# Sapphire-Bridge/rag-foundation

Hardware: AMD Instinct MI355X
Metric: top-k retrieval QPS + achieved HBM GB/s, 10M×768 k=10, 1/2/4/8 MI355X (higher is better)
Workload: dtype bf16; 1 GPU; cfg3: 10000000x768 bf16 corpus row-sharded over 1 GPU(s), 256 queries/batch, brute-force top-10; rows=10000000, dim=768, nq=256, k=10, parallelism=rowshard1, corpus_copies=1, scan=auto, exchange=none (one shard)

## Files before the change

rag-foundation_amd/csrc/k10_dbg.hip:

```cpp
#define RFX_K10_BLOCK_TIMES
#include "k_scan_screen64.h"

namespace rfx {
namespace k10q {
int launch_768(int kl, dim3 grid, hipStream_t st, const int8_t* X, const uint4* tm, const uint32_t* sts, const int8_t* Qc,
               const float* qe2, int nq, int ntiles, uint32_t* tau, float* cs, int* cr, uint32_t* dr, int64_t n_lists,
               const uint32_t* mask, uint32_t* xb, uint32_t* xw);
}

int launch_scan_screen_dbg(const MfmaPlan& p, int variant, const int8_t* X, const void* tmv, const uint32_t* sts,
                           int nrows, const int8_t* Qc, const float* qe2, int nq, uint32_t* tau, float* cs, int* cr,
                           uint32_t* dr, hipStream_t st) {
  const uint4* tm = (const uint4*)tmv;
  if (!p.ok || p.k_lane != 10) return -1;
  const int ntiles = (nrows + k10::kTM - 1) / k10::kTM;
  dim3 grid(p.blocks, p.q_blocks);
#define RFX_K10V(R, M)                                                                                        \
  case 100000000 * R + M:                                                                                          \
    hipLaunchKernelGGL((k10::scan_screen_kernel<10, 768, false, R, M>), grid, dim3(512), 0, st, X, tm, sts, Qc, \
                       qe2, nq, ntiles, tau, cs, cr, dr, p.n_lists, nullptr, tau + p.nq_pad * k10::kTauW,      \
                       xcd_weights_device_ptr());                                                             \
    break;
  switch (variant) {
    RFX_K10V(10, 2097152 + 8388608)
    RFX_K10V(10, 2097152 + 8388608 + 1)
    RFX_K10V(10, 2097152 + 8388608 + 9)
    RFX_K10V(10, 2097152 + 8388608 + 512)
    RFX_K10V(10, 2097152 + 8388608 + 8192)
    RFX_K10V(10, 2097152 + 8388608 + 65536)
    RFX_K10V(10, 2097152 + 8388608 + 33554432)
    case 64:
      if (p.lists_per_block != 1) return -1;
      return k10q::launch_768(10, grid, st, X, tm, sts, Qc, qe2, nq, ntiles, tau, cs, cr, dr, p.n_lists, nullptr,
                              tau + p.nq_pad * k10::kTauW, xcd_weights_device_ptr());
    case 65:
    case 73:
      if (p.lists_per_block != 1) return -1;
      if (variant == 65)
        hipLaunchKernelGGL((k10q::scan_screen_q64_kernel<10, 768, false, k10q::kRing768, 1>), grid, dim3(256), 0, st, X,
                           tm, sts, Qc, qe2, nq, ntiles, tau, cs, cr, dr, p.n_lists, nullptr, tau + p.nq_pad * k10::kTauW,
                           xcd_weights_device_ptr());
      else
        hipLaunchKernelGGL((k10q::scan_screen_q64_kernel<10, 768, false, k10q::kRing768, 9>), grid, dim3(256), 0, st, X,
                           tm, sts, Qc, qe2, nq, ntiles, tau, cs, cr, dr, p.n_lists, nullptr, tau + p.nq_pad * k10::kTauW,
                           xcd_weights_device_ptr());
      break;
    default:
      return -1;
  }
#undef RFX_K10V
  return 0;
}

int dbg_k10_trips(unsigned int* out_h, int reset) {
  if (reset) {
    static const unsigned int z[2][64] = {};
    return hipMemcpyToSymbol(HIP_SYMBOL(k10::g_k10_trips), z, sizeof(z)) == hipSuccess ? 0 : -1;
  }
  return hipMemcpyFromSymbol(out_h, HIP_SYMBOL(k10::g_k10_trips), sizeof(k10::g_k10_trips)) == hipSuccess ? 0 : -1;
}

int dbg_k10_block_times(unsigned long long* out_h) {
  return hipMemcpyFromSymbol(out_h, HIP_SYMBOL(k10::g_k10_bt), sizeof(k10::g_k10_bt)) == hipSuccess ? 0 : -1;
}

}
```

rag-foundation_amd/csrc/k_mfma_common.h:

```cpp
#pragma once
#include "rfx_device.h"
#include "rfx_kernels.h"

namespace rfx {
namespace mfc {

typedef __attribute__((ext_vector_type(8))) __bf16 v4bf16x8;
typedef __attribute__((ext_vector_type(8))) _Float16 v4f16x8;
typedef __attribute__((ext_vector_type(16))) float v4f32x16;

template <int DT>
__device__ __forceinline__ v4f32x16 mfma(const uint4& a, const uint4& b, const v4f32x16& c) {
  if constexpr (DT == RFX_BF16)
    return __builtin_amdgcn_mfma_f32_32x32x16_bf16(__builtin_bit_cast(v4bf16x8, a), __builtin_bit_cast(v4bf16x8, b),
                                                   c, 0, 0, 0);
  else
    return __builtin_amdgcn_mfma_f32_32x32x16_f16(__builtin_bit_cast(v4f16x8, a), __builtin_bit_cast(v4f16x8, b), c,
                                                  0, 0, 0);
}

typedef __attribute__((ext_vector_type(4))) float v4f32x4;
template <int DT>
__device__ __forceinline__ v4f32x4 mfma16(const uint4& a, const uint4& b, const v4f32x4& c) {
  if constexpr (DT == RFX_BF16)
    return __builtin_amdgcn_mfma_f32_16x16x32_bf16(__builtin_bit_cast(v4bf16x8, a), __builtin_bit_cast(v4bf16x8, b),
                                                   c, 0, 0, 0);
  else
    return __builtin_amdgcn_mfma_f32_16x16x32_f16(__builtin_bit_cast(v4f16x8, a), __builtin_bit_cast(v4f16x8, b), c,
                                                  0, 0, 0);
}

__device__ __forceinline__ uint32_t ord(float f) {
  const uint32_t b = __float_as_uint(f);
  return (b & 0x80000000u) ? ~b : (b | 0x80000000u);
}
__device__ __forceinline__ float unord(uint32_t o) {
  return __uint_as_float((o & 0x80000000u) ? (o & 0x7fffffffu) : ~o);
}
__device__ __forceinline__ float max3f(float a, float b, float c) { return fmaxf(fmaxf(a, b), c); }

typedef int v4i32 __attribute__((ext_vector_type(4)));

__device__ __forceinline__ v4i32 make_rsrc(const void* base) {
  const uint64_t a = (uint64_t)(uintptr_t)base;
  v4i32 d;
  d.x = __builtin_amdgcn_readfirstlane((int)(uint32_t)a);
  d.y = __builtin_amdgcn_readfirstlane((int)(uint32_t)(a >> 32) & 0xffff);
  d.z = -1;
  d.w = 0x00020000;
  return d;
}
__device__ __forceinline__ void bdma(v4i32 rsrc, uint32_t voff, uint32_t lds_addr) {
  asm volatile("s_nop 4\n\ts_mov_b32 m0, %2\n\ts_nop 0\n\tbuffer_load_dwordx4 %0, %1, 0 offen lds" ::"v"(voff), "s"(rsrc),
               "s"(lds_addr)
               : "memory", "m0");
}
__device__ __forceinline__ void bdma_nt(v4i32 rsrc, uint32_t voff, uint32_t lds_addr) {
  asm volatile("s_nop 4\n\ts_mov_b32 m0, %2\n\ts_nop 0\n\tbuffer_load_dwordx4 %0, %1, 0 offen nt lds" ::"v"(voff),
               "s"(rsrc), "s"(lds_addr)
               : "memory", "m0");
}
__device__ __forceinline__ void bdma_sc1(v4i32 rsrc, uint32_t voff, uint32_t lds_addr) {
  asm volatile("s_nop 4\n\ts_mov_b32 m0, %2\n\ts_nop 0\n\tbuffer_load_dwordx4 %0, %1, 0 offen sc1 lds" ::"v"(voff),
               "s"(rsrc), "s"(lds_addr)
               : "memory", "m0");
}
__device__ __forceinline__ void batomic_umax(v4i32 rsrc, uint32_t voff, uint32_t val) {
  asm volatile("s_nop 4\n\tbuffer_atomic_umax %0, %1, %2, 0 offen" ::"v"(val), "v"(voff), "s"(rsrc) : "memory");
}

__device__ __forceinline__ void glds(const void* src, uint32_t lds_addr) {
  asm volatile("s_mov_b32 m0, %1\n\ts_nop 0\n\tglobal_load_lds_dwordx4 %0, off" ::"v"(src), "s"(lds_addr)
               : "memory", "m0");
}
__device__ __forceinline__ void glds_sc1(const void* src, uint32_t lds_addr) {
  asm volatile("s_mov_b32 m0, %1\n\ts_nop 0\n\tglobal_load_lds_dwordx4 %0, off sc1" ::"v"(src), "s"(lds_addr)
               : "memory", "m0");
}

template <int N>
__device__ __forceinline__ void launder(uint4 (&v)[N]) {
#pragma unroll
  for (int i = 0; i < N; ++i) {
    v4i32 t = __builtin_bit_cast(v4i32, v[i]);
    asm volatile("" : "+v"(t));
    v[i] = __builtin_bit_cast(uint4, t);
  }
}

struct Acc4View {
  const v4f32x4 (&a)[4];
  __device__ __forceinline__ float operator[](int r) const { return a[r >> 2][r & 3]; }
};

template <int KL>
__device__ __forceinline__ uint32_t tau_min(const uint8_t* p) {
  const uint4 a = *(const uint4*)p;
  uint32_t m = min(min(a.x, a.y), min(a.z, a.w));
  if constexpr (KL > 4) {
    const uint4 b = *(const uint4*)(p + 16), c = *(const uint4*)(p + 32);
    m = min(m, min(min(b.x, b.y), min(b.z, b.w)));
    m = min(m, min(c.x, c.y));
  }
  return m;
}

template <int KL, int ROWMAP = 0, class V = v4f32x16>
__device__ __forceinline__ void fold(const V& acc, uint64_t* Ls, uint32_t& thr_o, int rbase, v4i32 tau_rsrc,
                                     uint32_t slot_voff, int& n_slow) {
  float mx = max3f(acc[0], acc[1], acc[2]);
#pragma unroll
  for (int r = 3; r < 15; r += 2) mx = max3f(mx, acc[r], acc[r + 1]);
  mx = fmaxf(mx, acc[15]);
  const float thr = thr_o ? unord(thr_o) : -__builtin_inff();
  if (mx >= thr) {
    ++n_slow;
#pragma unroll
    for (int r = 0; r < 16; ++r) {
      const float s = acc[r];
      if (s >= thr) {
        const int row = ROWMAP == 0   ? rbase + (r & 3) + 8 * (r >> 2)
                        : ROWMAP == 1 ? rbase + (r & 7) + 16 * (r >> 3)
                                      : rbase + (r & 3) + 16 * (r >> 2);
        const uint64_t key = ((uint64_t)ord(s) << 32) | (uint32_t)(~(uint32_t)row);
        if (key > Ls[(KL - 1) * 64]) {
          int i = KL - 1;
          for (; i > 0; --i) {
            const uint64_t prev = Ls[(i - 1) * 64];
            if (prev >= key) break;
            Ls[i * 64] = prev;
          }
          Ls[i * 64] = key;
        }
      }
    }
    const uint32_t own = (uint32_t)(Ls[(KL - 1) * 64] >> 32);
    thr_o = own > thr_o ? own : thr_o;
    batomic_umax(tau_rsrc, slot_voff, (uint32_t)(Ls[0] >> 32));
  }
}

}
}
```

rag-foundation_amd/csrc/k_scan_screen.h:

```cpp
#pragma once
#include "k_mfma_common.h"

namespace rfx {
namespace k10 {

using namespace mfc;

constexpr int kWaves = 8;
constexpr int kTM = 32;
constexpr int kQW = 32;
constexpr int kQG = kWaves * kQW;
constexpr int kQGSmall = 2 * kQW;
constexpr int kSK = 256;
constexpr int kRowB = kSK;
constexpr int kSlot = kTM * kRowB;
#ifndef RFX_K10_RING
#define RFX_K10_RING 8
#endif
constexpr int kRing = RFX_K10_RING;
constexpr int kGPW = 1;
constexpr int kTauW = 16;
constexpr int kTauBytes = kQG * kTauW * 4;
constexpr int kTauGPW = kTauBytes / 1024 / kWaves;
constexpr int kMR = 8;
constexpr int kXbWords = 8;
#ifdef RFX_K10_BLOCK_TIMES
__device__ unsigned long long g_k10_bt[1024][4];
__device__ unsigned int g_k10_trips[2][64];
#endif
template <int NW>
constexpr int tau_bytes_nw() { return NW * kQW * kTauW * 4; }
template <int RING>
constexpr int meta_off() { return RING * kSlot; }
template <int RING>
constexpr int tau_off() { return meta_off<RING>() + kMR * 1024; }
template <int RING, int NW = kWaves>
constexpr int list_off() { return tau_off<RING>() + tau_bytes_nw<NW>(); }
template <int KL, int RING, int NW = kWaves>
constexpr int ctr_off() { return list_off<RING, NW>(); }
template <int KL, int RING, int NW = kWaves>
constexpr int lds_bytes() { return list_off<RING, NW>() + (NW == kWaves ? kWaves * KL * 64 * 8 : 128); }
static_assert(lds_bytes<10, 12>() <= 163840, "LDS budget");
static_assert(2 * lds_bytes<16, 8, 2>() <= 163840, "two 2-wave workgroups per CU");

__device__ __forceinline__ void lds_spin_ge(const uint32_t* p, uint32_t target) {
  for (int guard = 0; guard < (1 << 20); ++guard) {
    if (__hip_atomic_load(p, __ATOMIC_RELAXED, __HIP_MEMORY_SCOPE_WORKGROUP) >= target) break;
    __builtin_amdgcn_s_sleep(1);
  }
}
__device__ __forceinline__ void lds_arrive(uint32_t* p) {
  __hip_atomic_fetch_add(p, 1u, __ATOMIC_RELAXED, __HIP_MEMORY_SCOPE_WORKGROUP);
}
static_assert(kSlot / 1024 == kWaves * kGPW && kTauGPW == 2, "DMA pieces per wave");

template <int MODE>
__device__ __forceinline__ bool tau_refresh_tile(int it) {
  return it < ((MODE & 16) != 0 ? 16 : 2) || (it & 3) == 3;
}

template <int KL>
__device__ __forceinline__ uint32_t kth16(uint32_t (&v)[16]) {
#pragma unroll
  for (int k = 2; k <= 16; k <<= 1)
#pragma unroll
    for (int j = k >> 1; j > 0; j >>= 1)
#pragma unroll
      for (int i = 0; i < 16; ++i) {
        const int l = i ^ j;
        if (l > i) {
          const uint32_t a = v[i], b = v[l];
          const bool desc = (i & k) == 0;
          v[i] = desc ? max(a, b) : min(a, b);
          v[l] = desc ? min(a, b) : max(a, b);
        }
      }
  return v[KL - 1];
}
template <int KL>
__device__ __forceinline__ uint32_t tau_kth(const uint8_t* p) {
  uint32_t v[16];
#pragma unroll
  for (int i = 0; i < 4; ++i) {
    const uint4 a = *(const uint4*)(p + 16 * i);
    v[4 * i] = a.x;
    v[4 * i + 1] = a.y;
    v[4 * i + 2] = a.z;
    v[4 * i + 3] = a.w;
  }
  return kth16<KL>(v);
}

__device__ __forceinline__ v4i32 mfma_i8(const uint4& a, const uint4& b, const v4i32& c) {
  return __builtin_amdgcn_mfma_i32_16x16x64_i8(__builtin_bit_cast(v4i32, a), __builtin_bit_cast(v4i32, b), c, 0, 0, 0);
}
__device__ __forceinline__ int max3i(int a, int b, int c) { return max(max(a, b), c); }

__device__ __forceinline__ uint32_t fold_mask(const v4i32 (&a)[4], float st, uint32_t bits, uint32_t thr_o, float e2,
                                              bool& pub) {
  int mx = max3i(a[0][0], a[0][1], a[0][2]);
  mx = max3i(mx, a[0][3], a[1][0]);
  mx = max3i(mx, a[1][1], a[1][2]);
  mx = max3i(mx, a[1][3], a[2][0]);
  mx = max3i(mx, a[2][1], a[2][2]);
  mx = max3i(mx, a[2][3], a[3][0]);
  mx = max3i(mx, a[3][1], a[3][2]);
  mx = max(mx, a[3][3]);
  const float thr = thr_o ? unord(thr_o) - e2 : -__builtin_inff();
  pub = (float)mx * st >= thr;
  uint32_t pm = 0;
  if (pub) {
#pragma unroll
    for (int r = 0; r < 16; ++r) pm |= (float)a[r >> 2][r & 3] * st >= thr ? (1u << r) : 0u;
    pm &= (bits & 0xffu) | ((bits >> 8) & 0xff00u);
  }
  return pm;
}
__device__ __forceinline__ uint32_t fold_mask_int(const v4i32 (&a)[4], float st, uint32_t bits, uint32_t thr_o, float e2,
                                                  bool& pub) {
  int mx = max3i(a[0][0], a[0][1], a[0][2]);
  mx = max3i(mx, a[0][3], a[1][0]);
  mx = max3i(mx, a[1][1], a[1][2]);
  mx = max3i(mx, a[1][3], a[2][0]);
  mx = max3i(mx, a[2][1], a[2][2]);
  mx = max3i(mx, a[2][3], a[3][0]);
  mx = max3i(mx, a[3][1], a[3][2]);
  mx = max(mx, a[3][3]);
  const float tf = thr_o ? unord(thr_o) - e2 : -__builtin_inff();
  constexpr int kBig = 1 << 30;
  int t;
  if (!(tf > -__builtin_inff())) {
    t = -kBig;
  } else if (!(st > 0.f)) {
    t = 0.f >= tf ? -kBig : kBig;
  } else {
    const float c = tf * __builtin_amdgcn_rcpf(st);
    const float cl = floorf(c - fabsf(c) * 0x1p-19f) - 2.f;
    t = (int)fminf(fmaxf(cl, -1073741824.f), 1073741824.f);
  }
  pub = mx >= t;
  uint32_t pm = 0;
  if (pub) {
    const int tm1 = t - 1;
#pragma unroll
    for (int r = 15; r >= 0; --r)
      pm = __builtin_amdgcn_alignbit(pm, (uint32_t)(tm1 - a[r >> 2][r & 3]), 31);
    pm &= (bits & 0xffu) | ((bits >> 8) & 0xff00u);
  }
  return pm;
}
template <int KL>
__device__ __forceinline__ void fold_trip(const v4i32 (&a)[4], float st, int rbase, uint32_t& pm, uint64_t (&L)[KL],
                                          uint32_t& drop_o) {
  const int r = __builtin_ctz(pm);
  pm &= pm - 1;
  int m3 = -((r >> 3) & 1), m2 = -((r >> 2) & 1), m1 = -((r >> 1) & 1), m0 = -(r & 1);
  asm volatile("" : "+v"(m3), "+v"(m2), "+v"(m1), "+v"(m0));
  int v[8];
#pragma unroll
  for (int j = 0; j < 8; ++j) v[j] = (a[(j + 8) >> 2][j & 3] & m3) | (a[j >> 2][j & 3] & ~m3);
#pragma unroll
  for (int j = 0; j < 4; ++j) v[j] = (v[j + 4] & m2) | (v[j] & ~m2);
#pragma unroll
  for (int j = 0; j < 2; ++j) v[j] = (v[j + 2] & m1) | (v[j] & ~m1);
  const int av = (v[1] & m0) | (v[0] & ~m0);
  const float s = (float)av * st;
  const int row = rbase + (r & 7) + 16 * (r >> 3);
  const uint64_t key = ((uint64_t)ord(s) << 32) | (uint32_t)(~(uint32_t)row);
  bool c[KL];
#pragma unroll
  for (int i = 0; i < KL; ++i) c[i] = L[i] > key;
  const uint64_t k = c[KL - 1] ? key : L[KL - 1];
#pragma unroll
  for (int i = KL - 1; i > 0; --i) L[i] = c[i - 1] ? (c[i] ? L[i] : key) : L[i - 1];
  L[0] = c[0] ? L[0] : key;
  drop_o = max(drop_o, (uint32_t)(k >> 32));
}
template <int KL, bool PUBCH = false>
__device__ __forceinline__ void fold_end(const uint64_t (&L)[KL], uint32_t& thr_o, bool pub, v4i32 tau_rsrc,
                                         uint32_t slot_voff, uint32_t& pubd) {
  if (pub) {
    const uint32_t own = (uint32_t)(L[KL - 1] >> 32);
    thr_o = own > thr_o ? own : thr_o;
    const uint32_t best = (uint32_t)(L[0] >> 32);
    if (!PUBCH || best > pubd) {
      batomic_umax(tau_rsrc, slot_voff, best);
      pubd = best;
    }
  }
}
__device__ __forceinline__ void cx_desc64(uint64_t& a, uint64_t& b) {
  const bool sw = a < b;
  const uint64_t hi = sw ? b : a, lo = sw ? a : b;
  a = hi;
  b = lo;
}
template <int N>
__device__ __forceinline__ void bitonic_desc64(uint64_t (&v)[N]) {
#pragma unroll
  for (int k = 2; k <= N; k <<= 1)
#pragma unroll
    for (int j = k >> 1; j > 0; j >>= 1)
#pragma unroll
      for (int i = 0; i < N; ++i) {
        const int l = i ^ j;
        if (l > i) {
          if ((i & k) == 0)
            cx_desc64(v[i], v[l]);
          else
            cx_desc64(v[l], v[i]);
        }
      }
}
template <int KL>
__device__ __forceinline__ void fold_sorted(const v4i32 (&a)[4], float st, int rbase, uint32_t pm, uint64_t (&L)[KL],
                                            uint32_t& drop_o) {
  static_assert(KL <= 16, "one 16-key merge");
  uint64_t K[16];
#pragma unroll
  for (int r = 0; r < 16; ++r) {
    const float s = (float)a[r >> 2][r & 3] * st;
    const int row = rbase + (r & 7) + 16 * (r >> 3);
    const uint64_t key = ((uint64_t)ord(s) << 32) | (uint32_t)(~(uint32_t)row);
    K[r] = (pm >> r) & 1u ? key : 0ull;
  }
  bitonic_desc64<16>(K);
  uint64_t M[16];
  uint32_t d = KL < 16 ? (uint32_t)(K[KL] >> 32) : 0u;
#pragma unroll
  for (int i = 0; i < KL; ++i) {
    const uint64_t x = L[i], y = K[KL - 1 - i];
    M[i] = x > y ? x : y;
    const uint64_t lo = x > y ? y : x;
    d = max(d, (uint32_t)(lo >> 32));
  }
#pragma unroll
  for (int i = KL; i < 16; ++i) M[i] = 0ull;
  bitonic_desc64<16>(M);
#pragma unroll
  for (int i = 0; i < KL; ++i) L[i] = M[i];
  drop_o = max(drop_o, d);
}
constexpr int kSortMergeTrips = 8;
template <int KL, bool REG = true, bool FMASK = false, bool SORTM = false, bool PUBCH = false>
__device__ __forceinline__ void fold_screen(const v4i32 (&a)[4], float st, uint32_t bits, uint64_t* Ls, uint64_t (&L)[KL],
                                            uint32_t& thr_o,
                                            float e2, uint32_t& drop_o, int rbase, v4i32 tau_rsrc, uint32_t slot_voff,
                                            uint32_t& pubd) {
  if constexpr (REG) {
    bool pub;
    uint32_t pm = FMASK ? fold_mask(a, st, bits, thr_o, e2, pub) : fold_mask_int(a, st, bits, thr_o, e2, pub);
    int many = 0;
    if constexpr (SORTM) {
      int c = __popc(pm);
#pragma unroll
      for (int off = 32; off; off >>= 1) c = max(c, __shfl_xor(c, off));
      many = c >= kSortMergeTrips;
    }
    if (SORTM && many) {
      fold_sorted<KL>(a, st, rbase, pm, L, drop_o);
    } else {
      while (pm) fold_trip<KL>(a, st, rbase, pm, L, drop_o);
    }
    fold_end<KL, PUBCH>(L, thr_o, pub, tau_rsrc, slot_voff, pubd);
  } else {
    const float thr = thr_o ? unord(thr_o) - e2 : -__builtin_inff();
#pragma unroll
    for (int r = 0; r < 16; ++r) {
      const float s = (float)a[r >> 2][r & 3] * st;
      if (((bits >> ((r & 7) + 16 * (r >> 3))) & 1u) && s >= thr) {
        const int row = rbase + (r & 7) + 16 * (r >> 3);
        const uint64_t key = ((uint64_t)ord(s) << 32) | (uint32_t)(~(uint32_t)row);
        const uint64_t last = Ls[(KL - 1) * 64];
        if (key > last) {
          if (last) drop_o = max(drop_o, (uint32_t)(last >> 32));
          int i = KL - 1;
          for (; i > 0; --i) {
            const uint64_t prev = Ls[(i - 1) * 64];
            if (prev >= key) break;
            Ls[i * 64] = prev;
          }
          Ls[i * 64] = key;
        } else {
          drop_o = max(drop_o, ord(s));
        }
      }
    }
    const uint32_t own = (uint32_t)(Ls[(KL - 1) * 64] >> 32);
    thr_o = own > thr_o ? own : thr_o;
    batomic_umax(tau_rsrc, slot_voff, (uint32_t)(Ls[0] >> 32));
  }
}

template <int KL>
__device__ __forceinline__ void insert_s(uint32_t (&S)[KL], uint32_t (&R)[KL], uint32_t key, uint32_t row,
                                         uint32_t& drop_o) {
  bool c[KL];
#pragma unroll
  for (int i = 0; i < KL; ++i) c[i] = S[i] >= key;
  drop_o = max(drop_o, min(S[KL - 1], key));
#pragma unroll
  for (int i = KL - 1; i > 0; --i) {
    R[i] = c[i] ? R[i] : (c[i - 1] ? row : R[i - 1]);
    S[i] = max(S[i], min(S[i - 1], key));
  }
  R[0] = c[0] ? R[0] : row;
  S[0] = max(S[0], key);
}
__device__ __forceinline__ int pass_threshold(float st, float tf, bool& ok) {
  auto P = [&](int d) { return (float)d * st >= tf; };
  if (!(tf > -__builtin_inff())) {
    ok = true;
    return INT_MIN;
  }
  if (!(st > 0.f)) {
    ok = true;
    return 0.f >= tf ? INT_MIN : INT_MAX;
  }
  const float c = tf * __builtin_amdgcn_rcpf(st);
  ok = fabsf(c) <= 4194304.f;
  int t = ok ? (int)ceilf(c) : 0;
  t -= P(t - 1) ? 1 : 0;
  t -= P(t - 1) ? 1 : 0;
  t += P(t) ? 0 : 1;
  t += P(t) ? 0 : 1;
  ok = ok && P(t) && !P(t - 1);
  return t;
}
__device__ __forceinline__ uint32_t pass_mask_int(const v4i32 (&a)[4], int t, uint32_t bits, uint32_t& all) {
  uint32_t pm = 0;
#pragma unroll
  for (int r = 0; r < 16; ++r) pm |= a[r >> 2][r & 3] >= t ? (1u << r) : 0u;
  all = pm;
  return pm & ((bits & 0xffu) | ((bits >> 8) & 0xff00u));
}

constexpr int kModeEpiLate = 131072;
constexpr int kModeStagger = 262144;
constexpr int kModePermBounds = 524288;
constexpr int kModeFold2 = 1048576;
constexpr int kModeTileBarrier = 2097152;
constexpr int kModeFloatMask = 4194304;
constexpr int kModePubOnChange = 8388608;
constexpr int kModeSortMerge = 16384;
constexpr int kModeMetaOne = 33554432;
template <int KL, int D, bool MASK, int RING = kRing, int MODE = 0, int NW = kWaves>
__global__ __launch_bounds__(64 * NW, 1) void scan_screen_kernel(const int8_t* __restrict__ X, const uint4* __restrict__ tmeta,
                                                             const uint32_t* __restrict__ stats,
                                                             const int8_t* __restrict__ Qc, const float* __restrict__ qe2,
                                                             int nq, int ntiles, uint32_t* __restrict__ tau,
                                                             float* __restrict__ cand_s, int* __restrict__ cand_r,
                                                             uint32_t* __restrict__ drops, int64_t n_lists,
                                                             const uint32_t* __restrict__ mask, uint32_t* __restrict__ xb,
                                                             uint32_t* __restrict__ xw) {
  constexpr int NKS = D / 64;
  constexpr int NST = D / kSK;
  constexpr int KPS = kSK / 64;
  static_assert(D % kSK == 0, "D must be a multiple of 256");
  static_assert(KL <= 16, "the bound is the KL-th largest of 16 slots");
  static_assert(NW == 8 || NW == 2, "8 waves (256 queries) or 2 waves (64 queries) per workgroup");
  constexpr int NT = 64 * NW;
  constexpr int QG = NW * kQW;
  constexpr int GPW = 8 / NW;
  constexpr int TAUB = tau_bytes_nw<NW>();
  static_assert(TAUB / 1024 / NW == kTauGPW, "slot-table DMA pieces per wave");
  __shared__ __attribute__((aligned(1024))) uint8_t lds[lds_bytes<KL, RING, NW>()];
  constexpr int kTauOff = tau_off<RING>();
  constexpr int kMetaOff = meta_off<RING>();
  constexpr int kListOff = list_off<RING, NW>();

  const int tid = threadIdx.x;
  const int w = tid >> 6, lane = tid & 63;
  const int half = lane >> 5;
  const int range = blockIdx.x;
  const int qg = blockIdx.y * QG;
  const int q = qg + w * kQW + 16 * ((lane >> 4) & 1) + (lane & 15);
  const int nblk = gridDim.x;
  const bool bal = (MODE & 4096) == 0 && xb != nullptr && xw != nullptr && (nblk & 7) == 0 && ntiles >= 64 * nblk;
  const int xc = range & 7;
  int tb0 = range, tstride = nblk, nt = range < ntiles ? (ntiles - range + nblk - 1) / nblk : 0;
  if (bal) {
    uint64_t pre = 0, tot = 0;
    uint32_t wx = 1;
#pragma unroll
    for (int x = 0; x < 8; ++x) {
      const uint32_t wv = xb[x];
      pre += x < xc ? wv : 0u;
      wx = x == xc ? wv : wx;
      tot += wv;
    }
    const int t_lo = (int)((uint64_t)ntiles * pre / tot), t_hi = (int)((uint64_t)ntiles * (pre + wx) / tot);
    const int bpx = nblk >> 3;
    tb0 = t_lo + (range >> 3);
    tstride = bpx;
    nt = tb0 < t_hi ? (t_hi - tb0 + bpx - 1) / bpx : 0;
  }
  auto tile_of = [&](int i) -> int { return tb0 + i * tstride; };
  const int S = nt * NST;
  const uint64_t t_start = wall_clock64();
  if (S == 0) return;
#ifdef RFX_K10_BLOCK_TIMES
  if constexpr ((MODE & 65536) != 0)
    if (tid == 0 && range < 1024 && blockIdx.y == 0) {
      g_k10_bt[range][0] = wall_clock64();
      g_k10_bt[range][2] = __builtin_amdgcn_s_memtime();
    }
#endif
  const int lst = range * 2 + half;
  const float e2 = qe2[q];
  const float smax = __uint_as_float(stats[2]);

  {
    uint4* tz = (uint4*)(lds + kTauOff);
#pragma unroll
    for (int i = 0; i < TAUB / 16 / NT; ++i) tz[tid + NT * i] = uint4{0u, 0u, 0u, 0u};
  }
  uint64_t* const Ls = (uint64_t*)(lds + kListOff) + (w * KL) * 64 + lane;
  if constexpr (NW == kWaves)
#pragma unroll
    for (int i = 0; i < KL; ++i) Ls[i * 64] = 0ull;
  uint32_t* const ready = (uint32_t*)(lds + ctr_off<KL, RING, NW>());
  uint32_t* const done = ready + 16;
  if (tid < 32) ready[tid] = 0u;
  constexpr bool F2 = (MODE & kModeFold2) != 0 && (MODE & 1024) == 0;
  constexpr bool SWEEP = D == 768;
  uint64_t Lr[KL];
  uint32_t LS[KL], LR[KL];
#pragma unroll
  for (int i = 0; i < KL; ++i) {
    Lr[i] = 0ull;
    LS[i] = 0u;
    LR[i] = 0u;
  }
  asm volatile("s_waitcnt lgkmcnt(0)" ::: "memory");
  __syncthreads();

  uint4 bq[2 * NKS];
#pragma unroll
  for (int qb = 0; qb < 2; ++qb) {
    const int8_t* qa = Qc + (int64_t)(qg + w * kQW + 16 * qb + (lane & 15)) * D + 16 * (lane >> 4);
#pragma unroll
    for (int ks = 0; ks < NKS; ++ks) bq[2 * ks + qb] = *(const uint4*)(qa + 64 * ks);
  }

  uint32_t laneoff[GPW];
#pragma unroll
  for (int u = 0; u < GPW; ++u) {
    const int pr = 4 * (w + NW * u) + (lane >> 4);
    laneoff[u] = (uint32_t)(pr * D + (((lane & 15) ^ (pr & 15)) * 16));
  }
  const uint32_t lds_base = (uint32_t)(uintptr_t)(__attribute__((address_space(3))) void*)lds;
  const v4i32 meta_rsrc = make_rsrc(tmeta);
  constexpr bool META1 = (MODE & kModeMetaOne) != 0 && (MODE & kModeTileBarrier) != 0 && (MODE & 32768) == 0 &&
                         (MODE & 8) == 0;
  auto issue_piece = [&](int gi, int slot) {
    const bool first = gi % NST == 0;
    gi = gi < S ? gi : S - 1;
    const int ti = gi / NST;
    const int si = gi - ti * NST;
    const int8_t* tbase = X + (int64_t)tile_of(ti) * kTM * D + si * kSK;
    const v4i32 rs = make_rsrc(tbase);
#pragma unroll
    for (int u = 0; u < GPW; ++u) {
      const uint32_t dst =
          __builtin_amdgcn_readfirstlane(lds_base + (uint32_t)(slot * kSlot) + (uint32_t)((w + NW * u) * 1024));
      bdma_nt(rs, laneoff[u], dst);
    }
    if (first && (!META1 || w == 0)) {
      const uint32_t mdst = __builtin_amdgcn_readfirstlane(lds_base + kMetaOff + (uint32_t)((ti % kMR) * 1024));
      bdma(meta_rsrc, (uint32_t)tile_of(ti) * 16u, mdst);
    }
  };
  const v4i32 tau_rsrc = make_rsrc(tau);
  auto issue_tau = [&]() {
#pragma unroll
    for (int u = 0; u < kTauGPW; ++u) {
      const int i = w + NW * u;
      const uint32_t dst = __builtin_amdgcn_readfirstlane(lds_base + kTauOff + i * 1024);
      bdma_sc1(tau_rsrc, (uint32_t)(qg * kTauW * 4 + tid * 16 + u * NW * 1024), dst);
    }
  };

  uint32_t thr = 0u, drop = 0u;
  uint32_t pubd = 0u;
  auto ibound = [&](uint32_t t_o) -> int {
    if (!t_o) return INT_MIN;
    const float tf = unord(t_o) - e2;
    if (!(tf > 0.f)) return INT_MIN;
    if (!(smax > 0.f)) return INT_MAX;
    const float qv = __fdiv_rn(tf, smax) * 0.999999f;
    return qv >= 2.0e9f ? INT_MAX : (int)floorf(qv);
  };
  int ti_own = INT_MIN, ti_oth = INT_MIN;
  const bool odd = ((lane >> 4) & 1) != 0;
  const bool qlive = q < nq;
  float tf_own = qlive ? -__builtin_inff() : __builtin_inff();
  float tf_oth = (odd ? q - 16 : q + 16) < nq ? -__builtin_inff() : __builtin_inff();
  auto set_bounds = [&]() {
    if constexpr ((MODE & 64) != 0) {
      ti_own = ibound(thr);
      ti_oth = __shfl_xor(ti_own, 16);
    } else {
      tf_own = !qlive ? __builtin_inff() : thr ? unord(thr) - e2 : -__builtin_inff();
      if constexpr ((MODE & kModePermBounds) != 0) {
        const uint32_t b = __float_as_uint(tf_own);
        const auto r = __builtin_amdgcn_permlane16_swap(b, b, false, false);
        tf_oth = __uint_as_float(odd ? r[0] : r[1]);
      } else {
        tf_oth = __shfl_xor(tf_own, 16);
      }
    }
  };
  if (xb != nullptr) {
    thr = xb[kXbWords + q];
    set_bounds();
  }
  constexpr int kSlots = (MODE & 256) != 0 ? KL : (MODE & 32) != 0 ? kTauW - 1 : kTauW;
  const uint32_t slot_voff = (uint32_t)(q * kTauW + lst % kSlots) * 4u;
  const uint8_t* const tq = lds + kTauOff + (w * kQW + (lane & 15) + 16 * ((lane >> 4) & 1)) * (kTauW * 4);
  const uint8_t* const frag_base = lds + (lane & 15) * kRowB;
  const int sw = lane & 15;
  struct Frag {
    uint4 a[2];
  };
  auto read_frag = [&](int slot, int kk) -> Frag {
    const uint8_t* p = frag_base + slot * kSlot + (((4 * kk + (lane >> 4)) ^ sw) << 4);
    Frag f;
    f.a[0] = *(const uint4*)p;
    f.a[1] = *(const uint4*)(p + 16 * kRowB);
    return f;
  };

  constexpr int PF = (D == 768 && (MODE & 4) == 0) ? 2 : 1;
  constexpr int NF = PF + 1;
  constexpr int KB = KPS - PF;
  constexpr bool DEC = (MODE & 32768) != 0 && (MODE & 8) == 0;
  constexpr int LAG = DEC ? 3 : 0;
  constexpr bool TB = (MODE & kModeTileBarrier) != 0 && !DEC && (MODE & 8) == 0;
  constexpr int AHEAD = TB ? RING - NST : RING - 1 - LAG;
  static_assert(!TB || RING >= 2 * NST + 2, "TB: at least two stages beyond the next tile in flight");
  constexpr int TBD = TB ? ((RING - NST + NST - 1) / NST > 2 ? (RING - NST + NST - 1) / NST : 2) : 2;
  constexpr int RA = AHEAD + 1;
  static_assert(AHEAD >= 3, "at least three stages in flight");
  constexpr int YNG = (RA - 2) * GPW;
  static_assert((NST * KPS) % NF == 0, "fragment rotation must realign every tile");

  asm volatile("s_waitcnt vmcnt(0)" ::: "memory");
  if constexpr ((MODE & 2) == 0) launder(bq);
  issue_tau();
#pragma unroll
  for (int p = 0; p < AHEAD; ++p) issue_piece(p, p);
  if constexpr (TB) {
    constexpr int NMT = (AHEAD - 1) / NST;
    if (META1 && w != 0)
      asm volatile("s_waitcnt vmcnt(%0)" ::"i"((AHEAD - NST) * GPW) : "memory");
    else
      asm volatile("s_waitcnt vmcnt(%0)" ::"i"((AHEAD - NST) * GPW + NMT) : "memory");
  } else {
    constexpr int NM0 = (AHEAD - 1) / NST + 1;
    asm volatile("s_waitcnt vmcnt(%0)" ::"i"(YNG + NM0) : "memory");
  }
  if constexpr (DEC)
    if (lane == 0) lds_arrive(&ready[0]);
  asm volatile("s_barrier" ::: "memory");

  Frag fr[NF];
#pragma unroll
  for (int p = 0; p < PF; ++p) fr[p] = read_frag(0, p);
  v4i32 accA[4], accB[4];
  auto epilogue = [&](const int it, v4i32(&acc4)[4]) {
    const int tile = tile_of(it);
    int m0 = max3i(acc4[0][0], acc4[0][1], acc4[0][2]);
    int m1 = max3i(acc4[1][0], acc4[1][1], acc4[1][2]);
    m0 = max3i(m0, acc4[0][3], acc4[2][0]);
    m1 = max3i(m1, acc4[1][3], acc4[3][0]);
    m0 = max3i(m0, acc4[2][1], acc4[2][2]);
    m1 = max3i(m1, acc4[3][1], acc4[3][2]);
    m0 = max(m0, acc4[2][3]);
    m1 = max(m1, acc4[3][3]);
    bool hit;
    if constexpr ((MODE & 64) != 0) {
      hit = (odd ? m1 : m0) >= ti_own || (odd ? m0 : m1) >= ti_oth;
    } else {
      const float st_t = *(const float*)(lds + kMetaOff + (it % kMR) * 1024 + lane * 16);
      hit = (float)(odd ? m1 : m0) * st_t >= tf_own || (float)(odd ? m0 : m1) * st_t >= tf_oth;
    }
    if constexpr ((MODE & 512) != 0) hit = hit && nq < 0;
    if constexpr ((MODE & 1) == 0) {
      if (__builtin_amdgcn_ballot_w64(hit)) {
        if constexpr ((MODE & 2048) != 0) __builtin_amdgcn_s_setprio(3);
        if constexpr ((MODE & 32) != 0)
          if (lane == 0) atomicAdd(tau + (int64_t)(qg + w * kQW) * kTauW + 15, 1u);
        const uint2 md = *(const uint2*)(lds + kMetaOff + (it % kMR) * 1024 + lane * 16);
        const float st = __uint_as_float(md.x);
        uint32_t lw = qlive ? md.y : 0u;
        if constexpr (MASK) lw &= mask[tile];
#pragma unroll
        for (int rb = 0; rb < 2; ++rb)
#pragma unroll
          for (int i = 0; i < 4; ++i) {
            const auto r = __builtin_amdgcn_permlane16_swap((uint32_t)acc4[2 * rb][i], (uint32_t)acc4[2 * rb + 1][i], false, false);
            acc4[2 * rb][i] = (int)r[0];
            acc4[2 * rb + 1][i] = (int)r[1];
          }
#ifdef RFX_K10_BLOCK_TIMES
        if constexpr ((MODE & 8192) != 0) {
          bool pub_;
          const uint32_t pm_ = (MODE & kModeFloatMask) != 0 ? fold_mask(acc4, st, lw >> (8 * half), thr, e2, pub_)
                                                             : fold_mask_int(acc4, st, lw >> (8 * half), thr, e2, pub_);
          int c = __popc(pm_);
#pragma unroll
          for (int off = 32; off; off >>= 1) c = max(c, __shfl_xor(c, off));
          if (lane == 0) {
            atomicAdd(&g_k10_trips[0][it < 63 ? it : 63], 1u);
            atomicAdd(&g_k10_trips[1][it < 63 ? it : 63], (unsigned)c);
          }
        }
#endif
        if constexpr (F2) {
          const uint32_t bits = lw >> (8 * half);
          const int rbase = tile * kTM + 8 * half;
          const float tf = thr ? unord(thr) - e2 : -__builtin_inff();
          bool ok;
          const int tq = pass_threshold(st, tf, ok);
          uint32_t all = 0, pm;
          if (__builtin_amdgcn_ballot_w64(!ok) == 0) {
            pm = pass_mask_int(acc4, tq, bits, all);
          } else {
            bool pubf;
            pm = fold_mask(acc4, st, bits, thr, e2, pubf);
            all = pubf ? 1u : 0u;
          }
          if (SWEEP && it < 2) {
#pragma unroll
            for (int r = 0; r < 16; ++r) {
              const float sv = (float)acc4[r >> 2][r & 3] * st;
              const uint32_t key = (pm >> r) & 1u ? ord(sv) : 0u;
              insert_s<KL>(LS, LR, key, (uint32_t)(rbase + (r & 7) + 16 * (r >> 3)), drop);
            }
          } else {
            while (pm) {
              const int r = __builtin_ctz(pm);
              pm &= pm - 1;
              int m3 = -((r >> 3) & 1), m2 = -((r >> 2) & 1), m1 = -((r >> 1) & 1), m0 = -(r & 1);
              asm volatile("" : "+v"(m3), "+v"(m2), "+v"(m1), "+v"(m0));
              int v[8];
#pragma unroll
              for (int j = 0; j < 8; ++j) v[j] = (acc4[(j + 8) >> 2][j & 3] & m3) | (acc4[j >> 2][j & 3] & ~m3);
#pragma unroll
              for (int j = 0; j < 4; ++j) v[j] = (v[j + 4] & m2) | (v[j] & ~m2);
#pragma unroll
              for (int j = 0; j < 2; ++j) v[j] = (v[j + 2] & m1) | (v[j] & ~m1);
              const int av = (v[1] & m0) | (v[0] & ~m0);
              insert_s<KL>(LS, LR, ord((float)av * st), (uint32_t)(rbase + (r & 7) + 16 * (r >> 3)), drop);
            }
          }
          if (all) {
            thr = LS[KL - 1] > thr ? LS[KL - 1] : thr;
            batomic_umax(tau_rsrc, slot_voff, LS[0]);
          }
        } else {
          fold_screen<KL, (MODE & 1024) == 0, (MODE & kModeFloatMask) != 0, (MODE & kModeSortMerge) != 0,
                      (MODE & kModePubOnChange) != 0>(
              acc4, st, lw >> (8 * half), Ls, Lr, thr, e2, drop,
                                                                              tile * kTM + 8 * half,
                                              tau_rsrc, slot_voff, pubd);
        }
        set_bounds();
        if constexpr ((MODE & 2048) != 0) __builtin_amdgcn_s_setprio(0);
      }
    } else if (hit && m0 == 12345 && m1 == 54321) {
      Ls[0] = 1;
    }
  };
  auto tile_body = [&](const int it, v4i32(&acc4)[4], v4i32(&accp)[4], const bool prev) {
    const int gbase = it * NST;
    if (it >= TBD && tau_refresh_tile<MODE>(it - TBD)) {
      thr = max(thr, (MODE & 256) != 0 ? tau_min<KL>(tq) : tau_kth<KL>(tq));
      set_bounds();
    }
    auto nmeta = [&](int s) {
      int c = 0;
#pragma unroll
      for (int j = 1; j <= RA - 1; ++j) c += (s + j) % NST == 0;
      return c;
    };
    auto young = [&](int s) {
      const int dmax = (RA - 3 + NST - s) / NST;
      bool y = false;
#pragma unroll
      for (int d = 1; d <= dmax; ++d) y = y || (it >= d && tau_refresh_tile<MODE>(it - d));
      return y;
    };
#pragma unroll
    for (int s = 0; s < NST; ++s) {
      const int g = gbase + s;
      const int slot = g % RING;
#pragma unroll
      for (int kk = 0; kk < KPS; ++kk) {
        if constexpr ((MODE & 8) == 0)
          if (kk == 0) {
            const int h = g + AHEAD;
            if constexpr (DEC)
              if (h >= RING) lds_spin_ge(&done[h % RING], (uint32_t)(8 * (h / RING)));
            issue_piece(h, h % RING);
          }
        if (kk == KB && TB) {
          if (s == NST - 1) {
            constexpr int NMY = (RING - NST - 1) / NST;
            int nt_ = 0;
#pragma unroll
            for (int d = 1; d <= TBD - 2; ++d) nt_ += (it >= d && tau_refresh_tile<MODE>(it - d)) ? kTauGPW : 0;
            static_assert(kTauGPW == 2, "wait table below");
            if (META1 && w != 0) {
              switch (nt_) {
#define RFX_K10_TWAIT(N)                                                                                      \
  case N:                                                                                                     \
    asm volatile("s_waitcnt vmcnt(%0) lgkmcnt(0)" ::"i"((RING - 2 * NST) * GPW + N) : "memory");               \
    break;
                RFX_K10_TWAIT(0) RFX_K10_TWAIT(2)
                default:
                  asm volatile("s_waitcnt vmcnt(%0) lgkmcnt(0)" ::"i"((RING - 2 * NST) * GPW) : "memory");
#undef RFX_K10_TWAIT
              }
            } else {
              switch (nt_) {
#define RFX_K10_TWAIT(N)                                                                                      \
  case N:                                                                                                     \
    asm volatile("s_waitcnt vmcnt(%0) lgkmcnt(0)" ::"i"((RING - 2 * NST) * GPW + NMY + N) : "memory");         \
    break;
                RFX_K10_TWAIT(0) RFX_K10_TWAIT(2)
                default:
                  asm volatile("s_waitcnt vmcnt(%0) lgkmcnt(0)" ::"i"((RING - 2 * NST) * GPW + NMY) : "memory");
#undef RFX_K10_TWAIT
              }
            }
            asm volatile("s_barrier" ::: "memory");
            if (tau_refresh_tile<MODE>(it)) issue_tau();
          }
        } else if (kk == KB) {
          if constexpr ((MODE & 8) == 0) {
            const int nm = nmeta(s) + (young(s) ? kTauGPW : 0);
            static_assert(kTauGPW == 2 && RA <= 13, "wait table below covers nm <= 6");
            switch (nm) {
#define RFX_K10_WAIT(N)                                                                  \
  case N:                                                                                \
    asm volatile("s_waitcnt vmcnt(%0) lgkmcnt(0)" ::"i"(YNG + N) : "memory");            \
    break;
              RFX_K10_WAIT(0) RFX_K10_WAIT(1) RFX_K10_WAIT(2) RFX_K10_WAIT(3) RFX_K10_WAIT(4) RFX_K10_WAIT(5)
              default:
                asm volatile("s_waitcnt vmcnt(%0) lgkmcnt(0)" ::"i"(YNG + 6) : "memory");
#undef RFX_K10_WAIT
            }
          } else {
            asm volatile("s_waitcnt lgkmcnt(0)" ::: "memory");
          }
          if constexpr (DEC) {
            if (lane == 0) {
              lds_arrive(&done[g % RING]);
              lds_arrive(&ready[(g + 1) % RING]);
            }
            if (s == NST - 1 && tau_refresh_tile<MODE>(it)) issue_tau();
            if (g + 1 < S) lds_spin_ge(&ready[(g + 1) % RING], (uint32_t)(8 * ((g + 1) / RING + 1)));
          } else {
            asm volatile("s_barrier" ::: "memory");
            if constexpr ((MODE & 8) == 0)
              if (s == NST - 1 && tau_refresh_tile<MODE>(it)) issue_tau();
          }
        }
        const int ks = s * KPS + kk;
        fr[(ks + PF) % NF] = kk + PF < KPS ? read_frag(slot, kk + PF) : read_frag((g + 1) % RING, kk + PF - KPS);
        const Frag& cur = fr[ks % NF];
        __builtin_amdgcn_sched_group_barrier(0x100, 2, 0);
        __builtin_amdgcn_sched_group_barrier(0x008, 4, 0);
#pragma unroll
        for (int rb = 0; rb < 2; ++rb)
#pragma unroll
          for (int qb = 0; qb < 2; ++qb)
            acc4[2 * rb + qb] = ks == 0 ? mfma_i8(cur.a[rb], bq[2 * ks + qb], v4i32{0, 0, 0, 0})
                                        : mfma_i8(cur.a[rb], bq[2 * ks + qb], acc4[2 * rb + qb]);
        if constexpr ((MODE & 128) == 0) {
          constexpr int EK = (MODE & kModeEpiLate) != 0 ? KB : 0;
          if (kk == EK && prev) {
            if constexpr ((MODE & kModeStagger) != 0 && NST >= 2) {
              if (s == 0 && w < 4) epilogue(it - 1, accp);
              if (s == 1 && w >= 4) epilogue(it - 1, accp);
            } else {
              if (s == 0) epilogue(it - 1, accp);
            }
          }
        }
      }
    }

  };
  if constexpr ((MODE & 128) != 0) {
    for (int it = 0; it < nt; ++it) {
      tile_body(it, accA, accB, false);
      epilogue(it, accA);
    }
  } else {
    int it = 0;
    for (; it + 1 < nt; it += 2) {
      tile_body(it, accA, accB, it > 0);
      tile_body(it + 1, accB, accA, true);
    }
    if (it < nt) {
      tile_body(it, accA, accB, it > 0);
      epilogue(it, accA);
    } else {
      epilogue(it - 1, accB);
    }
  }
  asm volatile("s_waitcnt vmcnt(0)" ::: "memory");
  if (q < nq) {
    uint32_t sl[16];
#pragma unroll
    for (int j = 0; j < 16; ++j)
      sl[j] = j >= kSlots ? 0u : __hip_atomic_load(tau + (int64_t)q * kTauW + j, __ATOMIC_RELAXED, __HIP_MEMORY_SCOPE_AGENT);
    uint32_t m = kth16<KL>(sl);
    if constexpr ((MODE & 256) != 0) {
      m = 0xffffffffu;
#pragma unroll
      for (int j = 0; j < KL; ++j)
        m = min(m, __hip_atomic_load(tau + (int64_t)q * kTauW + j, __ATOMIC_RELAXED, __HIP_MEMORY_SCOPE_AGENT));
    }
    const uint32_t fin = max(thr, m);
    const float lo = fin ? unord(fin) - e2 : -__builtin_inff();
    const int64_t o = ((int64_t)q * n_lists + lst) * KL;
#pragma unroll
    for (int i = 0; i < KL; ++i) {
      const uint64_t key = F2 ? (((uint64_t)LS[i] << 32) | (uint32_t)~LR[i]) : (MODE & 1024) == 0 ? Lr[i] : Ls[i * 64];
      const float sc = unord((uint32_t)(key >> 32));
      const bool keep = (key >> 32) != 0 && sc >= lo;
      cand_s[o + i] = keep ? sc : -__builtin_inff();
      cand_r[o + i] = keep ? (int)(~(uint32_t)key) : kEmptyRow;
    }
    drops[(int64_t)q * n_lists + lst] = drop;
  }
  if (bal && blockIdx.y == 0 && tid == 0) {
    const uint64_t dt = wall_clock64() - t_start;
    __hip_atomic_fetch_add(xw + 8 + xc, (uint32_t)(dt < 0xffffffull ? dt : 0xffffffull), __ATOMIC_RELAXED,
                           __HIP_MEMORY_SCOPE_AGENT);
    __hip_atomic_fetch_add(xw + 16 + xc, (uint32_t)nt, __ATOMIC_RELAXED, __HIP_MEMORY_SCOPE_AGENT);
  }
#ifdef RFX_K10_BLOCK_TIMES
  if constexpr ((MODE & 65536) != 0) {
    asm volatile("s_waitcnt vmcnt(0)" ::: "memory");
    __syncthreads();
    if (tid == 0 && range < 1024 && blockIdx.y == 0) {
      g_k10_bt[range][1] = wall_clock64();
      g_k10_bt[range][3] = __builtin_amdgcn_s_memtime();
    }
  }
#endif
}

constexpr int kProdRing = 10;
constexpr int kProdMode = kModeTileBarrier | kModePubOnChange;
template <int D>
constexpr int w2_ring() { return 8; }
template <int D>
constexpr int w2_mode() { return D == 768 ? kProdMode : kModePubOnChange; }
#define RFX_K10_INSTANTIATE_W2(DV, NAME)                                                                      \
  int NAME(int kl, dim3 grid, hipStream_t st, const int8_t* X, const uint4* tm, const uint32_t* sts,           \
           const int8_t* Qc, const float* qe2, int nq, int ntiles, uint32_t* tau, float* cs, int* cr,          \
           uint32_t* dr, int64_t n_lists, const uint32_t* mask, uint32_t* xb, uint32_t* xw) {               \
    constexpr int R = w2_ring<DV>(), M = w2_mode<DV>();                                                     \
    if (kl == 4 && !mask)                                                                                   \
      hipLaunchKernelGGL((scan_screen_kernel<4, DV, false, R, M, 2>), grid, dim3(128), 0, st, X, tm, sts, Qc,  \
                         qe2, nq, ntiles, tau, cs, cr, dr, n_lists, mask, xb, xw);                           \
    else if (kl == 10 && !mask)                                                                             \
      hipLaunchKernelGGL((scan_screen_kernel<10, DV, false, R, M, 2>), grid, dim3(128), 0, st, X, tm, sts, Qc, \
                         qe2, nq, ntiles, tau, cs, cr, dr, n_lists, mask, xb, xw);                           \
    else if (kl == 4)                                                                                       \
      hipLaunchKernelGGL((scan_screen_kernel<4, DV, true, R, M, 2>), grid, dim3(128), 0, st, X, tm, sts, Qc,   \
                         qe2, nq, ntiles, tau, cs, cr, dr, n_lists, mask, xb, xw);                           \
    else if (kl == 10)                                                                                      \
      hipLaunchKernelGGL((scan_screen_kernel<10, DV, true, R, M, 2>), grid, dim3(128), 0, st, X, tm, sts, Qc,  \
                         qe2, nq, ntiles, tau, cs, cr, dr, n_lists, mask, xb, xw);                           \
    else                                                                                                    \
      return -1;                                                                                            \
    return 0;                                                                                               \
  }

#define RFX_K10_INSTANTIATE(DV, NAME)                                                                         \
  int NAME(int kl, dim3 grid, hipStream_t st, const int8_t* X, const uint4* tm, const uint32_t* sts,           \
           const int8_t* Qc, const float* qe2, int nq, int ntiles, uint32_t* tau, float* cs, int* cr,          \
           uint32_t* dr, int64_t n_lists, const uint32_t* mask, uint32_t* xb, uint32_t* xw) {               \
    if (kl == 4 && !mask)                                                                                   \
      hipLaunchKernelGGL((scan_screen_kernel<4, DV, false, kProdRing, kProdMode>), grid, dim3(512), 0, st, X, tm, sts, Qc, qe2, nq,   \
                         ntiles, tau, cs, cr, dr, n_lists, mask, xb, xw);                                    \
    else if (kl == 10 && !mask)                                                                             \
      hipLaunchKernelGGL((scan_screen_kernel<10, DV, false, kProdRing, kProdMode>), grid, dim3(512), 0, st, X, tm, sts, Qc, qe2, nq,  \
                         ntiles, tau, cs, cr, dr, n_lists, mask, xb, xw);                                    \
    else if (kl == 4)                                                                                       \
      hipLaunchKernelGGL((scan_screen_kernel<4, DV, true, kProdRing, kProdMode>), grid, dim3(512), 0, st, X, tm, sts, Qc, qe2, nq,    \
                         ntiles, tau, cs, cr, dr, n_lists, mask, xb, xw);                                    \
    else if (kl == 10)                                                                                      \
      hipLaunchKernelGGL((scan_screen_kernel<10, DV, true, kProdRing, kProdMode>), grid, dim3(512), 0, st, X, tm, sts, Qc, qe2, nq,   \
                         ntiles, tau, cs, cr, dr, n_lists, mask, xb, xw);                                    \
    else                                                                                                    \
      return -1;                                                                                            \
    return 0;                                                                                               \
  }

}
}
```

Before: 119,000 queries/s.

## Add lean scan modes: running DMA cursor, precomputed LDS offsets, faster screen, thinner tau refresh

Adds four mode bits to the int8 MFMA screening scan kernel and turns them on in the production modes. The first streams corpus tiles through a running buffer resource with a scalar offset instead of recomputing per-piece addresses. The second precomputes per-lane LDS fragment offsets with a rotating ring offset. The third precomputes the odd/even threshold selection for the screen test, and the fourth refreshes tau less often after the first 64 tiles. The goal is to cut address and select ALU overhead in the hot loop. The price is staler pruning thresholds, which may let more candidates through, plus extra register pressure.

```diff
diff --git a/rag-foundation_amd/csrc/k10_dbg.hip b/rag-foundation_amd/csrc/k10_dbg.hip
--- a/rag-foundation_amd/csrc/k10_dbg.hip
+++ b/rag-foundation_amd/csrc/k10_dbg.hip
@@ -29,6 +29,17 @@
     RFX_K10V(10, 2097152 + 8388608 + 8192)
     RFX_K10V(10, 2097152 + 8388608 + 65536)
     RFX_K10V(10, 2097152 + 8388608 + 33554432)
+    RFX_K10V(10, 2097152 + 8388608 + 32)
+    RFX_K10V(10, 2097152 + 8388608 + 268435456 + 32)
+    RFX_K10V(10, 2097152 + 8388608 + 536870912 + 32)
+    RFX_K10V(10, 2097152 + 8388608 + 67108864)
+    RFX_K10V(10, 2097152 + 8388608 + 134217728)
+    RFX_K10V(10, 2097152 + 8388608 + 67108864 + 134217728 + 16777216)
+    RFX_K10V(10, 2097152 + 8388608 + 268435456)
+    RFX_K10V(10, 2097152 + 8388608 + 67108864 + 268435456)
+    RFX_K10V(10, 2097152 + 8388608 + 67108864 + 134217728 + 16777216 + 268435456)
+    RFX_K10V(10, 2097152 + 8388608 + 67108864 + 134217728 + 16777216 + 536870912)
+    RFX_K10V(10, 2097152 + 8388608 + 67108864 + 134217728 + 16777216 + 268435456 + 512)
     case 64:
       if (p.lists_per_block != 1) return -1;
       return k10q::launch_768(10, grid, st, X, tm, sts, Qc, qe2, nq, ntiles, tau, cs, cr, dr, p.n_lists, nullptr,
diff --git a/rag-foundation_amd/csrc/k10_stream.h b/rag-foundation_amd/csrc/k10_stream.h
--- /dev/null
+++ b/rag-foundation_amd/csrc/k10_stream.h
@@ -0,0 +1,50 @@
+#pragma once
+#include <cstdint>
+
+#if defined(__HIPCC__) || defined(__CUDACC__)
+#define RFX_K10S_HD __host__ __device__ __forceinline__
+#else
+#define RFX_K10S_HD inline
+#endif
+
+namespace rfx {
+namespace k10s {
+
+constexpr int kTileRows = 32;
+constexpr int kStageB = 256;
+constexpr int kMetaSlots = 8;
+constexpr int kRecB = 16;
+
+struct TileCursor {
+  uint64_t code_byte;
+  uint32_t rec_byte;
+  uint32_t mslot;
+  int ti;
+};
+
+RFX_K10S_HD TileCursor cursor_at(int ti, int tb0, int tstride, int D) {
+  const int64_t tile = (int64_t)tb0 + (int64_t)ti * tstride;
+  TileCursor c;
+  c.code_byte = (uint64_t)tile * (uint64_t)(kTileRows * D);
+  c.rec_byte = (uint32_t)tile * (uint32_t)kRecB;
+  c.mslot = (uint32_t)ti % (uint32_t)kMetaSlots;
+  c.ti = ti;
+  return c;
+}
+
+RFX_K10S_HD void cursor_next_tile(TileCursor& c, int nt, int tstride, int D) {
+  if (c.ti + 1 < nt) {
+    ++c.ti;
+    c.code_byte += (uint64_t)(uint32_t)tstride * (uint64_t)(kTileRows * D);
+    c.rec_byte += (uint32_t)tstride * (uint32_t)kRecB;
+    c.mslot = (c.mslot + 1u) & (uint32_t)(kMetaSlots - 1);
+  }
+}
+
+RFX_K10S_HD uint32_t ring_next(uint32_t off, uint32_t slot_bytes, uint32_t ring_bytes) {
+  const uint32_t n = off + slot_bytes;
+  return n == ring_bytes ? 0u : n;
+}
+
+}
+}
diff --git a/rag-foundation_amd/csrc/k_mfma_common.h b/rag-foundation_amd/csrc/k_mfma_common.h
--- a/rag-foundation_amd/csrc/k_mfma_common.h
+++ b/rag-foundation_amd/csrc/k_mfma_common.h
@@ -58,6 +58,11 @@
 __device__ __forceinline__ void bdma_nt(v4i32 rsrc, uint32_t voff, uint32_t lds_addr) {
   asm volatile("s_nop 4\n\ts_mov_b32 m0, %2\n\ts_nop 0\n\tbuffer_load_dwordx4 %0, %1, 0 offen nt lds" ::"v"(voff),
                "s"(rsrc), "s"(lds_addr)
+               : "memory", "m0");
+}
+__device__ __forceinline__ void bdma_nt_soff(v4i32 rsrc, uint32_t voff, uint32_t soff, uint32_t lds_addr) {
+  asm volatile("s_mov_b32 m0, %3\n\ts_nop 3\n\tbuffer_load_dwordx4 %0, %1, %2 offen nt lds" ::"v"(voff), "s"(rsrc),
+               "s"(soff), "s"(lds_addr)
                : "memory", "m0");
 }
 __device__ __forceinline__ void bdma_sc1(v4i32 rsrc, uint32_t voff, uint32_t lds_addr) {
diff --git a/rag-foundation_amd/csrc/k_scan_screen.h b/rag-foundation_amd/csrc/k_scan_screen.h
--- a/rag-foundation_amd/csrc/k_scan_screen.h
+++ b/rag-foundation_amd/csrc/k_scan_screen.h
@@ -1,5 +1,6 @@
 #pragma once
 #include "k_mfma_common.h"
+#include "k10_stream.h"
 
 namespace rfx {
 namespace k10 {
@@ -54,8 +55,14 @@
 }
 static_assert(kSlot / 1024 == kWaves * kGPW && kTauGPW == 2, "DMA pieces per wave");
 
+constexpr int kThinBit = 268435456, kThin64Bit = 536870912;
+constexpr int kThinFrom = 64;
 template <int MODE>
 __device__ __forceinline__ bool tau_refresh_tile(int it) {
+  if constexpr ((MODE & (kThinBit | kThin64Bit)) != 0) {
+    const int m = it < kThinFrom ? 3 : ((MODE & kThin64Bit) != 0 ? 63 : 15);
+    return it < ((MODE & 16) != 0 ? 16 : 2) || (it & m) == m;
+  }
   return it < ((MODE & 16) != 0 ? 16 : 2) || (it & 3) == 3;
 }
 
@@ -344,6 +351,11 @@
 constexpr int kModePubOnChange = 8388608;
 constexpr int kModeSortMerge = 16384;
 constexpr int kModeMetaOne = 33554432;
+constexpr int kModeFastSel = 16777216;
+constexpr int kModeRunAddr = 67108864;
+constexpr int kModeFragOff = 134217728;
+constexpr int kModeThin = kThinBit;
+constexpr int kModeThin64 = kThin64Bit;
 template <int KL, int D, bool MASK, int RING = kRing, int MODE = 0, int NW = kWaves>
 __global__ __launch_bounds__(64 * NW, 1) void scan_screen_kernel(const int8_t* __restrict__ X, const uint4* __restrict__ tmeta,
                                                              const uint32_t* __restrict__ stats,
@@ -371,6 +383,7 @@
 
   const int tid = threadIdx.x;
   const int w = tid >> 6, lane = tid & 63;
+  const int wu = __builtin_amdgcn_readfirstlane(w);
   const int half = lane >> 5;
   const int range = blockIdx.x;
   const int qg = blockIdx.y * QG;
@@ -496,6 +509,8 @@
   const bool qlive = q < nq;
   float tf_own = qlive ? -__builtin_inff() : __builtin_inff();
   float tf_oth = (odd ? q - 16 : q + 16) < nq ? -__builtin_inff() : __builtin_inff();
+  constexpr bool FSEL = (MODE & kModeFastSel) != 0 && (MODE & 64) == 0;
+  float tf_m0 = odd ? tf_oth : tf_own, tf_m1 = odd ? tf_own : tf_oth;
   auto set_bounds = [&]() {
     if constexpr ((MODE & 64) != 0) {
       ti_own = ibound(thr);
@@ -508,6 +523,10 @@
         tf_oth = __uint_as_float(odd ? r[0] : r[1]);
       } else {
         tf_oth = __shfl_xor(tf_own, 16);
+      }
+      if constexpr (FSEL) {
+        tf_m0 = odd ? tf_oth : tf_own;
+        tf_m1 = odd ? tf_own : tf_oth;
       }
     }
   };
@@ -531,6 +550,22 @@
     return f;
   };
 
+  constexpr bool FOFF = (MODE & kModeFragOff) != 0;
+  uint32_t foff[KPS];
+#pragma unroll
+  for (int kk = 0; kk < KPS; ++kk) {
+    foff[kk] = (uint32_t)((lane & 15) * kRowB + (((4 * kk + (lane >> 4)) ^ sw) << 4));
+    if constexpr (FOFF) asm volatile("" : "+v"(foff[kk]));
+  }
+  auto read_frag_o = [&](uint32_t slot_off, int kk) -> Frag {
+    const uint8_t* p = lds + (foff[kk] + slot_off);
+    Frag f;
+    f.a[0] = *(const uint4*)p;
+    f.a[1] = *(const uint4*)(p + 16 * kRowB);
+    return f;
+  };
+  uint32_t rd_off = 0u, rd_nxt = RING > 1 ? (uint32_t)kSlot : 0u;
+
   constexpr int PF = (D == 768 && (MODE & 4) == 0) ? 2 : 1;
   constexpr int NF = PF + 1;
   constexpr int KB = KPS - PF;
@@ -563,6 +598,23 @@
   if constexpr (DEC)
     if (lane == 0) lds_arrive(&ready[0]);
   asm volatile("s_barrier" ::: "memory");
+
+  constexpr bool RUN = (MODE & kModeRunAddr) != 0 && (MODE & 8) == 0;
+  k10s::TileCursor cur = k10s::cursor_at(min((AHEAD - 1) / NST, nt - 1), tb0, tstride, D);
+  v4i32 run_rs = make_rsrc(X + cur.code_byte);
+  uint32_t wr_off = (uint32_t)((AHEAD % RING) * kSlot);
+  const uint32_t wdst0 = lds_base + (uint32_t)(wu * 1024);
+  auto issue_run = [&](const int si) {
+    if (si == 0) {
+      k10s::cursor_next_tile(cur, nt, tstride, D);
+      run_rs = make_rsrc(X + cur.code_byte);
+    }
+#pragma unroll
+    for (int u = 0; u < GPW; ++u)
+      bdma_nt_soff(run_rs, laneoff[u], (uint32_t)(si * kSK), wdst0 + wr_off + (uint32_t)(NW * u * 1024));
+    if (si == 0 && (!META1 || w == 0)) bdma(meta_rsrc, cur.rec_byte, lds_base + kMetaOff + cur.mslot * 1024u);
+    wr_off = k10s::ring_next(wr_off, kSlot, RING * kSlot);
+  };
 
   Frag fr[NF];
 #pragma unroll
@@ -583,7 +635,10 @@
       hit = (odd ? m1 : m0) >= ti_own || (odd ? m0 : m1) >= ti_oth;
     } else {
       const float st_t = *(const float*)(lds + kMetaOff + (it % kMR) * 1024 + lane * 16);
-      hit = (float)(odd ? m1 : m0) * st_t >= tf_own || (float)(odd ? m0 : m1) * st_t >= tf_oth;
+      if constexpr (FSEL)
+        hit = (float)m0 * st_t >= tf_m0 || (float)m1 * st_t >= tf_m1;
+      else
+        hit = (float)(odd ? m1 : m0) * st_t >= tf_own || (float)(odd ? m0 : m1) * st_t >= tf_oth;
     }
     if constexpr ((MODE & 512) != 0) hit = hit && nq < 0;
     if constexpr ((MODE & 1) == 0) {
@@ -703,7 +758,10 @@
             const int h = g + AHEAD;
             if constexpr (DEC)
               if (h >= RING) lds_spin_ge(&done[h % RING], (uint32_t)(8 * (h / RING)));
-            issue_piece(h, h % RING);
+            if constexpr (RUN)
+              issue_run((s + AHEAD) % NST);
+            else
+              issue_piece(h, h % RING);
           }
         if (kk == KB && TB) {
           if (s == NST - 1) {
@@ -769,16 +827,19 @@
           }
         }
         const int ks = s * KPS + kk;
-        fr[(ks + PF) % NF] = kk + PF < KPS ? read_frag(slot, kk + PF) : read_frag((g + 1) % RING, kk + PF - KPS);
-        const Frag& cur = fr[ks % NF];
+        if constexpr (FOFF)
+          fr[(ks + PF) % NF] = kk + PF < KPS ? read_frag_o(rd_off, kk + PF) : read_frag_o(rd_nxt, kk + PF - KPS);
+        else
+          fr[(ks + PF) % NF] = kk + PF < KPS ? read_frag(slot, kk + PF) : read_frag((g + 1) % RING, kk + PF - KPS);
+        const Frag& cf = fr[ks % NF];
         __builtin_amdgcn_sched_group_barrier(0x100, 2, 0);
         __builtin_amdgcn_sched_group_barrier(0x008, 4, 0);
 #pragma unroll
         for (int rb = 0; rb < 2; ++rb)
 #pragma unroll
           for (int qb = 0; qb < 2; ++qb)
-            acc4[2 * rb + qb] = ks == 0 ? mfma_i8(cur.a[rb], bq[2 * ks + qb], v4i32{0, 0, 0, 0})
-                                        : mfma_i8(cur.a[rb], bq[2 * ks + qb], acc4[2 * rb + qb]);
+            acc4[2 * rb + qb] = ks == 0 ? mfma_i8(cf.a[rb], bq[2 * ks + qb], v4i32{0, 0, 0, 0})
+                                        : mfma_i8(cf.a[rb], bq[2 * ks + qb], acc4[2 * rb + qb]);
         if constexpr ((MODE & 128) == 0) {
           constexpr int EK = (MODE & kModeEpiLate) != 0 ? KB : 0;
           if (kk == EK && prev) {
@@ -791,6 +852,10 @@
           }
         }
       }
+      if constexpr (FOFF) {
+        rd_off = rd_nxt;
+        rd_nxt = k10s::ring_next(rd_nxt, kSlot, RING * kSlot);
+      }
     }
 
   };
@@ -857,11 +922,12 @@
 }
 
 constexpr int kProdRing = 10;
-constexpr int kProdMode = kModeTileBarrier | kModePubOnChange;
+constexpr int kLeanMode = kModeRunAddr | kModeFragOff | kModeFastSel | kModeThin;
+constexpr int kProdMode = kModeTileBarrier | kModePubOnChange | kLeanMode;
 template <int D>
 constexpr int w2_ring() { return 8; }
 template <int D>
-constexpr int w2_mode() { return D == 768 ? kProdMode : kModePubOnChange; }
+constexpr int w2_mode() { return D == 768 ? kProdMode : (kModePubOnChange | kLeanMode); }
 #define RFX_K10_INSTANTIATE_W2(DV, NAME)                                                                      \
   int NAME(int kl, dim3 grid, hipStream_t st, const int8_t* X, const uint4* tm, const uint32_t* sts,           \
            const int8_t* Qc, const float* qe2, int nq, int ntiles, uint32_t* tau, float* cs, int* cr,          \
```

Result: faster. 127,500 queries/s, median of 6 (+7.1%).
